# ilVecc/AquaticGymEnv

Hardware: AMD Instinct MI355X
Metric: env-steps/sec at batch=262144; achieved HBM GB/s vs roofline; 1/2/4/8-GPU scaling (higher is better)
Workload: dtype f32

## Files before the change

### aquaticgymenv_amd/csrc/aqua_hip.hip

```cpp
#include <hip/hip_runtime.h>
#include <hip/hip_ext.h>

#include <cmath>
#include <cstdarg>
#include <cstddef>
#include <type_traits>
#include <cstdio>
#include <cstring>
#include <vector>

#include "../../include/aqua_hip.h"
#include "aqua_device.hpp"

using namespace aqua;

namespace {

constexpr int TILE_WORLDS = 1024;
constexpr int BLOCK_SMALL = 256;
constexpr int RESET_GROUP = 8;
constexpr int MAX_GRID = 1 << 30;

constexpr size_t AQUA_BLOB_MIN_BYTES = 320;

struct StepArgs {
    float* state;
    int64_t ld;
    int32_t* time;
    const void* action;
    int64_t action_ld;
    const float* noise;
    int64_t noise_ld;
    float* reward;
    uint8_t* term;
    uint64_t* done_bits;
    float* obs_norm;
    const void* obst_blob;
    const uint64_t* tick_base;
    uint64_t seed, tick;
    int64_t N, env_offset;
    int64_t T, action_step_stride, out_step_stride;
    int64_t reseed_blocks;
    int K, waves, time_limit, auto_reset, random_boat, random_goal;
    float W, sigma;
    uint64_t* tick_copy_to;
    uint64_t* tick_bump_to;
    uint64_t tick_bump;
};

struct NsArgs {
    float* row[7];
    int32_t* time;
    const void* action;
    float* reward;
    uint8_t* term;
    uint64_t* done_bits;
    const void* obst_blob;
    const uint64_t* tick_base;
    uint64_t seed, tick;
    int64_t env_offset;
    uint32_t N, reseed_blocks;
    int32_t K, time_limit;
    float W, sigma;
    uint32_t flags;
    uint32_t reserved;
    const float* action_hi;
    const float* noise[2];
    float* norm[5];
    uint64_t* tick_copy_to;
    uint64_t* tick_bump_to;
    uint64_t tick_bump;
};
enum : uint32_t { NS_WAVES_MASK = 0xFFu, NS_RANDOM_BOAT = 1u << 8, NS_RANDOM_GOAL = 1u << 9, NS_HAS_NOISE = 1u << 10,
                  NS_HAS_NORM = 1u << 11, NS_DONE_WORD_WB = 1u << 12 };
constexpr int64_t NS_LAUNCH_MAX_WORLDS = int64_t(1) << 28;

__device__ __forceinline__ int args_waves(const StepArgs& a) { return a.waves; }
__device__ __forceinline__ int args_waves(const NsArgs& a) { return static_cast<int>(a.flags & NS_WAVES_MASK); }
__device__ __forceinline__ int args_random_boat(const StepArgs& a) { return a.random_boat; }
__device__ __forceinline__ int args_random_boat(const NsArgs& a) { return (a.flags & NS_RANDOM_BOAT) != 0; }
__device__ __forceinline__ int args_random_goal(const StepArgs& a) { return a.random_goal; }
__device__ __forceinline__ int args_random_goal(const NsArgs& a) { return (a.flags & NS_RANDOM_GOAL) != 0; }

template <typename T>
__device__ __forceinline__ T ld1(const T* p)
{
    return *p;
}
template <typename T>
__device__ __forceinline__ void st1(T* p, T v, bool wb = false)
{
#ifdef AQUA_ST1_PLAIN
    *p = v;
#else
    if (wb) *p = v;
    else __hip_atomic_store(p, v, __ATOMIC_RELAXED, __HIP_MEMORY_SCOPE_AGENT);
#endif
}

constexpr int64_t STORE_WB_SAME_STEP_MIN = int64_t(1) << 21;
constexpr int64_t STORE_WB_NEXT_STEP_MIN = int64_t(1) << 21, STORE_WB_NEXT_STEP_MAX = 3 * (int64_t(1) << 22);

constexpr int64_t DONE_WORD_WRITE_THROUGH_MAX_WORLDS = int64_t(1) << 20;
__device__ __forceinline__ void store_done_word(uint64_t* p, uint64_t v, int64_t n_worlds)
{
    if (n_worlds <= DONE_WORD_WRITE_THROUGH_MAX_WORLDS) st1(p, v);
    else *p = v;
}

template <typename T>
__device__ __forceinline__ T ld_at(const T* base, uint32_t byte_off)
{
    return ld1(reinterpret_cast<const T*>(reinterpret_cast<const char*>(base) + byte_off));
}
template <typename T>
__device__ __forceinline__ void st_at(T* base, uint32_t byte_off, T v, bool wb = false)
{
    st1(reinterpret_cast<T*>(reinterpret_cast<char*>(base) + byte_off), v, wb);
}

__device__ __forceinline__ ObstPtr obstacle_rows(const void* blob)
{
    return (ObstPtr)(uintptr_t)(static_cast<const char*>(blob) + sizeof(ObstHeader));
}

template <int QUICK = QUICK_NEVER, typename A>
__device__ __forceinline__ StepConst make_const(const A& a, ObstPtr obst)
{
    StepConst k;
    k.quick = nullptr;
    k.W = a.W; k.sigma = a.sigma; k.waves = args_waves(a); k.time_limit = a.time_limit; k.K = a.K;
    k.obst = obst;
    k.Kc = 0; k.band2 = 0.0f; k.band2_tight = 0.0f;
    k.touch[0] = k.touch[1] = k.touch[2] = k.touch[3] = 0;
    if (a.obst_blob != nullptr) {
        const ObstHeader __attribute__((address_space(4)))* h =
            (const ObstHeader __attribute__((address_space(4)))*)(uintptr_t)a.obst_blob;
        k.Kc = h->n_circles;
        k.band2 = h->band2;
        k.band2_tight = h->band2_tight;
        const uint32_t __attribute__((address_space(4)))* w = (const uint32_t __attribute__((address_space(4)))*)(uintptr_t)a.obst_blob;
        if (QUICK == QUICK_ALWAYS || (QUICK == QUICK_IF_PRESENT && a.K <= QUICK_MAX)) {
            k.quick = (QuickPtr)(uintptr_t)(reinterpret_cast<const char*>(a.obst_blob) + quick_offset(a.K));
            k.qc0 = quick_circles(k.quick, QUICK_C0);
            k.qr0 = quick_rects(k.quick, QUICK_R0);
        }
        k.touch[0] = w[16]; k.touch[1] = w[32]; k.touch[2] = w[48]; k.touch[3] = w[64];
    }
    k.obst64 = reinterpret_cast<const double*>(reinterpret_cast<const char*>(a.obst_blob) + sizeof(ObstHeader) +
                                               sizeof(ObstF) * a.K);
    return k;
}

__device__ __forceinline__ int fold_index(int64_t a)
{
    if (a < 0) a += 3;
    return a < 0 ? 0 : (a > 2 ? 2 : static_cast<int>(a));
}

struct Motion {
    float h, w, chord;
    float vl, vr;
    int idx;
};

// ... 448 lines not shown
    if (lane == 0) sh.count[parity][wave] = static_cast<uint32_t>(__builtin_popcountll(m));
    __syncthreads();
    uint32_t first = 0, total = 0;
#pragma unroll
    for (int w = 0; w < WAVES; ++w) {
        const uint32_t c = sh.count[parity][w];
        if (w < wave) first += c;
        total += c;
    }
    return ReseedTicket{uni(total), first + pos};
}

template <bool SMALL, typename A>
__device__ __forceinline__ void serve_reseed(const ReseedTicket& tk, const A& a, const StepConst& k, uint64_t tick,
                                             int64_t block_first_world, RolloutShared& sh, int parity)
{
    constexpr int WAVES = BLOCK_SMALL / 64;
    const int wave = threadIdx.x >> 6, lane = threadIdx.x & 63;
    if (tk.n == 0 || wave != static_cast<int>((static_cast<uint32_t>(tick) + blockIdx.x) & (WAVES - 1))) return;
#ifdef AQUA_FUSED_NOSERVE
    return;
#endif
    uint32_t first[WAVES + 1];
    first[0] = 0;
#pragma unroll
    for (int w = 0; w < WAVES; ++w) first[w + 1] = first[w] + sh.count[parity][w];
    constexpr uint32_t PER_PASS = 64 / RESET_GROUP;
    for (uint32_t qb = 0; qb < tk.n; qb += PER_PASS) {
        const uint32_t q = qb + (lane / RESET_GROUP);
        const bool active = q < tk.n;
        uint32_t seg = 0;
#pragma unroll
        for (int w = 1; w < WAVES; ++w) seg += (active && q >= first[w]) ? 1u : 0u;
        const uint32_t owner = sh.list[parity][seg][active ? q - first[seg] : 0];
        const uint64_t world = static_cast<uint64_t>(a.env_offset + block_first_world) + owner;
        EnvState f;
        if constexpr (SMALL)
            f = reset_env_group<RESET_GROUP, RESEED_QUICK>(active, a.seed, world, tick, k.waves, args_random_boat(a), args_random_goal(a),
                                                        k.K, k.obst, nullptr, k.quick, k.Kc);
        else
            f = reset_env_group<RESET_GROUP>(active, a.seed, world, tick, k.waves, args_random_boat(a), args_random_goal(a), k.K, k.obst);
        if (active && (lane & (RESET_GROUP - 1)) == 0) {
            float* r = sh.result[q];
            r[0] = f.x; r[1] = f.y; r[2] = f.th; r[3] = f.gx; r[4] = f.gy; r[5] = f.wx; r[6] = f.wy;
        }
    }
}

__device__ __forceinline__ void collect_reseed(EnvState& e, bool need, const ReseedTicket& tk, RolloutShared& sh)
{
    if (tk.n == 0) return;
    __syncthreads();
    if (need) {
        const float* r = sh.result[tk.slot];
        e.x = r[0]; e.y = r[1]; e.th = r[2]; e.gx = r[3]; e.gy = r[4]; e.wx = r[5]; e.wy = r[6]; e.t = 0;
    }
}

#ifndef AQUA_FUSED_MAIL
#define AQUA_FUSED_MAIL 1
#endif
#ifndef AQUA_MAIL_SPIN_LIMIT
#define AQUA_MAIL_SPIN_LIMIT (1u << 18)
#endif
constexpr uint32_t MAIL_SPIN_LIMIT = AQUA_MAIL_SPIN_LIMIT;
#ifndef AQUA_MAIL_PRIO
#define AQUA_MAIL_PRIO 2
#endif
struct RolloutMail {
    uint32_t posted[BLOCK_SMALL / 64];
    uint32_t served;
    uint32_t count[2][BLOCK_SMALL / 64];
    uint8_t list[2][BLOCK_SMALL / 64][64];
    float result[2][BLOCK_SMALL][8];
};

__device__ __forceinline__ uint32_t lds_offset(const void* p)
{
    return static_cast<uint32_t>(reinterpret_cast<uintptr_t>((const __attribute__((address_space(3))) void*)p));
}
__device__ __forceinline__ void mail_wait(const uint32_t* flag, uint32_t at_least)
{
    const uint32_t at = lds_offset(flag);
    for (uint32_t polls = 0; polls < MAIL_SPIN_LIMIT; ++polls) {
        uint32_t v;
        asm volatile("ds_read_b32 %0, %1\n\ts_waitcnt lgkmcnt(0)" : "=v"(v) : "v"(at) : "memory");
        if (uni(v) >= at_least) break;
        __builtin_amdgcn_s_sleep(1);
    }
}
__device__ __forceinline__ void mail_flag(uint32_t* flag, uint32_t value)
{
    asm volatile("s_waitcnt lgkmcnt(0)\n\tds_write_b32 %0, %1" ::"v"(lds_offset(flag)), "v"(value) : "memory");
}
__device__ __forceinline__ uint32_t mail_post(bool need, RolloutMail& sh, uint32_t q)
{
    const int wave = threadIdx.x >> 6, lane = threadIdx.x & 63, parity = static_cast<int>(q & 1u);
    if (q >= 2u) mail_wait(&sh.served, q - 1u);
    const uint64_t m = __ballot(need);
    const uint32_t pos = __builtin_amdgcn_mbcnt_hi(static_cast<uint32_t>(m >> 32), __builtin_amdgcn_mbcnt_lo(static_cast<uint32_t>(m), 0u));
    if (need) sh.list[parity][wave][pos] = static_cast<uint8_t>(lane);
    if (lane == 0) {
        sh.count[parity][wave] = static_cast<uint32_t>(__builtin_popcountll(m));
        mail_flag(&sh.posted[wave], q + 1u);
    }
    return pos;
}

template <bool SMALL, typename A>
__device__ __forceinline__ void mail_serve(const A& a, const StepConst& k, uint64_t tick, int64_t block_first_world, RolloutMail& sh, uint32_t q)
{
    constexpr int WAVES = BLOCK_SMALL / 64;
    const int lane = threadIdx.x & 63, parity = static_cast<int>(q & 1u);
    uint32_t first[WAVES + 1];
    first[0] = 0;
#pragma unroll
    for (int w = 0; w < WAVES; ++w) {
        mail_wait(&sh.posted[w], q + 1u);
        first[w + 1] = first[w] + sh.count[parity][w];
    }
#ifdef AQUA_FUSED_NOSERVE
    const uint32_t n = 0;
#else
    const uint32_t n = uni(first[WAVES]);
#endif
    constexpr uint32_t PER_PASS = 64 / RESET_GROUP;
    for (uint32_t qb = 0; qb < n; qb += PER_PASS) {
        const uint32_t i = qb + (lane / RESET_GROUP);
        const bool active = i < n;
        uint32_t seg = 0;
#pragma unroll
        for (int w = 1; w < WAVES; ++w) seg += (active && i >= first[w]) ? 1u : 0u;
        const uint32_t at = active ? i - first[seg] : 0u;
        const uint32_t owner = seg * 64u + sh.list[parity][seg][at];
        const uint64_t world = static_cast<uint64_t>(a.env_offset + block_first_world) + owner;
        EnvState f;
        if constexpr (SMALL)
            f = reset_env_group<RESET_GROUP, RESEED_QUICK>(active, a.seed, world, tick, k.waves, args_random_boat(a), args_random_goal(a),
                                                        k.K, k.obst, nullptr, k.quick, k.Kc);
        else
            f = reset_env_group<RESET_GROUP>(active, a.seed, world, tick, k.waves, args_random_boat(a), args_random_goal(a), k.K, k.obst);
        if (active && (lane & (RESET_GROUP - 1)) == 0) {
            float* r = sh.result[parity][seg * 64u + at];
            r[0] = f.x; r[1] = f.y; r[2] = f.th; r[3] = f.gx; r[4] = f.gy; r[5] = f.wx; r[6] = f.wy;
        }
    }
    if (lane == 0) mail_flag(&sh.served, q + 1u);
}

__device__ __forceinline__ void mail_collect(EnvState& e, bool need, uint32_t pos, RolloutMail& sh, uint32_t q)
{
    if (!any_lane(need)) return;
    mail_wait(&sh.served, q + 1u);
    if (need) {
        const float* r = sh.result[q & 1u][(threadIdx.x & ~63u) + pos];
        e.x = r[0]; e.y = r[1]; e.th = r[2]; e.gx = r[3]; e.gy = r[4]; e.wx = r[5]; e.wy = r[6];
    }
}

struct TileShared {
    uint32_t count[TILE_WORLDS / 64];
    uint16_t list[TILE_WORLDS / 64][64];
};

template <int AK, bool SMALL_TABLE, bool RESTART, bool WB = false>
__global__ __launch_bounds__(TILE_WORLDS) void step_kernel(const NsArgs a)
// ... 43 lines not shown
    }
    asm volatile("" : "+v"(tin[0]), "+v"(u0[0]), "+v"(u1[0]));
    hold_loads<1, AK>(x, y, th, gx, gy, wx, wy, araw, avl, avr);
    fold_actions<1, AK>(araw, aidx);
    if constexpr (AK == AQUA_ACT_BEARING) aidx[0] = bearing_action(x[0], y[0], th[0], gx[0], gy[0]);
    const float x0 = x[0], y0 = y[0], th0 = th[0], wx0 = wx[0], wy0 = wy[0];
    EnvState e{x[0], y[0], th[0], gx[0], gy[0], wx[0], wy[0], tin[0]};
    const Motion mo = decode_motion<AK>(k, aidx[0], avl[0], avr[0]);
    float rew;
    uint32_t code;
    asm volatile("" ::"s"(k.touch[0]), "s"(k.touch[1]), "s"(k.touch[2]), "s"(k.touch[3]));
    const bool knife = fast_step<false, QUICK>(e, mo.h, mo.w, mo.chord, u0[0], u1[0], k, rew, code) && valid;
    if (__builtin_expect(any_lane(knife), 0)) {
        if (knife) {
            const ExactOut o2 = exact_step(x0, y0, th0, gx[0], gy[0], wx0, wy0, e.t, exact_motion<AK>(mo), k.K, k.obst64,
                                           k.obst, k.band2, k.time_limit);
            e.x = o2.x; e.y = o2.y; e.th = o2.th; rew = o2.reward; code = o2.term;
        }
    }
    const bool done = valid && code != 0u;
    uint32_t s4 = o4, s1 = o;
    asm volatile("" : "+v"(s4), "+v"(s1));
    constexpr bool wb = WB;
    if (valid) {
        st_at(a.reward, s4, rew, wb);
        st_at(a.term, s1, static_cast<uint8_t>(code), wb);
    }
    const uint64_t done_ballot = __ballot(done);
    if (a.done_bits != nullptr) {
        const uint32_t word = (tile >> 6) + (uni(off) >> 6);
        if (word < ((a.N + 63u) >> 6) && lane == 0) {
            if (a.flags & NS_DONE_WORD_WB) a.done_bits[word] = done_ballot;
            else st1(a.done_bits + word, done_ballot);
        }
    }
    if (valid && !(RESTART && done)) {
        st_at(a.row[0], s4, e.x, wb); st_at(a.row[1], s4, e.y, wb); st_at(a.row[2], s4, e.th, wb);
        st_at(a.row[5], s4, e.wx, wb); st_at(a.row[6], s4, e.wy, wb);
        st_at(a.time, s4, e.t, wb);
        ns_write_norm(a, s4, e.x, e.y, e.th, gx[0], gy[0], wb);
    }
    if constexpr (RESTART) {
        __shared__ TileShared sh;
        constexpr int WAVES = TILE_WORLDS / 64;
        if (done) sh.list[wave][__builtin_amdgcn_mbcnt_hi(static_cast<uint32_t>(done_ballot >> 32),
                                __builtin_amdgcn_mbcnt_lo(static_cast<uint32_t>(done_ballot), 0u))] = static_cast<uint16_t>(off);
        if (lane == 0) sh.count[wave] = static_cast<uint32_t>(__builtin_popcountll(done_ballot));
        __syncthreads();
        uint32_t first[WAVES + 1];
        first[0] = 0;
#pragma unroll
        for (int w = 0; w < WAVES; ++w) first[w + 1] = first[w] + sh.count[w];
        const uint32_t n_done = uni(first[WAVES]);
        const int waves = args_waves(a), random_boat = args_random_boat(a), random_goal = args_random_goal(a);
        const uint64_t env_base = static_cast<uint64_t>(a.env_offset) + tile;
        constexpr uint32_t GROUPS = TILE_WORLDS / RESET_GROUP;
        for (uint32_t qb = static_cast<uint32_t>(wave) * (64 / RESET_GROUP); qb < n_done; qb += GROUPS) {
            const uint32_t q = qb + (lane / RESET_GROUP);
            const bool active = q < n_done;
            uint32_t seg = 0;
#pragma unroll
            for (int w = 1; w < WAVES; ++w) seg += (active && q >= first[w]) ? 1u : 0u;
            const uint32_t i = sh.list[seg][active ? q - first[seg] : 0];
            EnvState f;
            if constexpr (SMALL_TABLE)
                f = reset_env_group<RESET_GROUP, RESEED_QUICK>(active, a.seed, env_base + i, tick, waves, random_boat, random_goal,
                                                            k.K, k.obst, nullptr, k.quick, k.Kc);
            else
                f = reset_env_group<RESET_GROUP>(active, a.seed, env_base + i, tick, waves, random_boat, random_goal, k.K, k.obst);
            if (active && (lane & (RESET_GROUP - 1)) == 0) {
                const uint32_t i4 = (tile + i) * 4u;
                st_at(a.row[0], i4, f.x, wb); st_at(a.row[1], i4, f.y, wb); st_at(a.row[2], i4, f.th, wb);
                st_at(a.row[3], i4, f.gx, wb); st_at(a.row[4], i4, f.gy, wb);
                st_at(a.row[5], i4, f.wx, wb); st_at(a.row[6], i4, f.wy, wb);
                st_at(a.time, i4, f.t, wb);
                ns_write_norm(a, i4, f.x, f.y, f.th, f.gx, f.gy, wb);
            }
        }
    }
}

constexpr bool rollout_mail(int mode) { return AQUA_FUSED_MAIL && mode == AQUA_RESET_NEXT_STEP; }
constexpr int rollout_threads(int mode) { return rollout_mail(mode) ? BLOCK_SMALL + 64 : BLOCK_SMALL; }
template <int AK, bool SMALL, int MODE>
__global__ __launch_bounds__(rollout_threads(MODE), rollout_threads(MODE) / 64) void rollout_kernel(const StepArgs a)
{
    constexpr bool MAIL = rollout_mail(MODE);
    __shared__ typename std::conditional<MAIL, RolloutMail, RolloutShared>::type sh;
    if constexpr (MAIL) {
        if (threadIdx.x < BLOCK_SMALL / 64) sh.posted[threadIdx.x] = 0u;
        if (threadIdx.x == 0) sh.served = 0u;
        __syncthreads();
    }
    constexpr int QUICK = SMALL ? QUICK_ALWAYS : QUICK_NEVER;
    const uint64_t tick0 = launch_tick(a);
    const int64_t N = a.N, ld = a.ld;
    uint32_t q0 = 0;
    if constexpr (MAIL) {
        if (threadIdx.x >= BLOCK_SMALL) {
            StepConst k = make_const<QUICK_NEVER>(a, obstacle_rows(a.obst_blob));
            if constexpr (SMALL) k.quick = (QuickPtr)(uintptr_t)(reinterpret_cast<const char*>(a.obst_blob) + quick_offset(a.K));
            if (AQUA_MAIL_PRIO) __builtin_amdgcn_s_setprio(AQUA_MAIL_PRIO);
            for (int64_t bbase = static_cast<int64_t>(blockIdx.x) * BLOCK_SMALL; bbase < N;
                 bbase += static_cast<int64_t>(gridDim.x) * BLOCK_SMALL, q0 += static_cast<uint32_t>(a.T))
                for (int64_t p = 0; p < a.T; ++p)
                    mail_serve<SMALL>(a, k, tick0 + static_cast<uint64_t>(p), bbase, sh, q0 + static_cast<uint32_t>(p));
            return;
        }
    }
#ifdef AQUA_FUSED_QUICK_RESIDENT
    const StepConst k = make_const<SMALL ? QUICK_IF_PRESENT : QUICK_NEVER>(a, obstacle_rows(a.obst_blob));
#else
    StepConst k = make_const<QUICK_NEVER>(a, obstacle_rows(a.obst_blob));
    if constexpr (SMALL) k.quick = (QuickPtr)(uintptr_t)(reinterpret_cast<const char*>(a.obst_blob) + quick_offset(a.K));
#endif
    for (int64_t bbase = static_cast<int64_t>(blockIdx.x) * BLOCK_SMALL; bbase < N;
         bbase += static_cast<int64_t>(gridDim.x) * BLOCK_SMALL, q0 += static_cast<uint32_t>(a.T)) {
        const int64_t i = bbase + threadIdx.x;
        const bool valid = i < N;
        const int64_t ic = valid ? i : N - 1;
        EnvState e{a.state[0 * ld + ic], a.state[1 * ld + ic], a.state[2 * ld + ic], a.state[3 * ld + ic],
                   a.state[4 * ld + ic], a.state[5 * ld + ic], a.state[6 * ld + ic], a.time[ic]};
        const uint64_t env = static_cast<uint64_t>(a.env_offset + i);
        bool owed = false;
        uint32_t owed_pos = 0, posted_pos = 0;
        if constexpr (MAIL) posted_pos = mail_post(valid && e.t == done_code(tick0 - 1), sh, q0);
        for (int64_t s = 0; s < a.T; ++s) {
            const uint64_t tick = tick0 + static_cast<uint64_t>(s);
            const int parity = static_cast<int>(s & 1);
            bool pending = false, restart = false;
            ReseedTicket tk{0u, 0u};
            if constexpr (MODE == AQUA_RESET_NEXT_STEP) {
                if (e.t == restart_code(tick - 1)) e.t = 0;
                restart = valid && e.t == done_code(tick - 1);
                pending = valid && e.t < 0;
                if constexpr (!MAIL) {
                    tk = publish_reseed(restart, sh, parity);
                    serve_reseed<SMALL>(tk, a, k, tick, bbase, sh, parity);
                }
            }
            int idx = 2;
            float vl = 0.5f, vr = 0.5f;
            if constexpr (AK == AQUA_ACT_U8) idx = fold_index(static_cast<const uint8_t*>(a.action)[s * a.action_step_stride + ic]);
            if constexpr (AK == AQUA_ACT_I32) idx = fold_index(static_cast<const int32_t*>(a.action)[s * a.action_step_stride + ic]);
            if constexpr (AK == AQUA_ACT_I64) idx = fold_index(static_cast<const int64_t*>(a.action)[s * a.action_step_stride + ic]);
            if constexpr (AK == AQUA_ACT_F32X2) {
                const float* base = static_cast<const float*>(a.action) + s * a.action_step_stride;
                vl = base[ic]; vr = base[a.action_ld + ic];
            }
            uint64_t seed = a.seed;
#ifdef AQUA_FUSED_KEYS_LAUNDERED
            asm volatile("" : "+s"(seed));
#endif
            uint32_t w0[1], w1[1];
            pair_draws<1, false>(seed, env, tick, STREAM_STEP, w0, w1);
            const float u0 = u_pm1(w0[0]), u1 = u_pm1(w1[0]);
            if constexpr (AK >= AQUA_ACT_SAMPLE_D) {
                pair_draws<1, false>(seed, env, tick, STREAM_ACT, w0, w1);
                if constexpr (AK == AQUA_ACT_SAMPLE_D) idx = sample_discrete(w0[0]);
                else { vl = sample_thrust(w0[0]); vr = sample_thrust(w1[0]); }
            }
            if constexpr (MAIL) {
                if (s > 0) mail_collect(e, owed, owed_pos, sh, q0 + static_cast<uint32_t>(s) - 1u);
            }
            if constexpr (AK == AQUA_ACT_BEARING) idx = bearing_action(e.x, e.y, e.th, e.gx, e.gy);
            const Motion m = decode_motion<AK>(k, idx, vl, vr);
            const EnvState before = e;
            EnvState after = e;
            float rew;
            uint32_t code;
#ifndef AQUA_FUSED_QUICK_RESIDENT
            if constexpr (SMALL) {
                QuickPtr q = k.quick;
                asm volatile("" : "+s"(q));
                k.qc0 = quick_circles(q, QUICK_C0);
                k.qr0 = quick_rects(q, QUICK_R0);
            }
#endif
            const bool knife = fast_step<false, QUICK>(after, m.h, m.w, m.chord, u0, u1, k, rew, code) && valid && !pending;
            if (__builtin_expect(any_lane(knife), 0)) {
                if (knife) {
                    const ExactOut o = exact_step(before.x, before.y, before.th, before.gx, before.gy, before.wx,
                                                  before.wy, after.t, exact_motion<AK>(m), k.K, k.obst64, k.obst, k.band2,
                                                  k.time_limit);
                    after.x = o.x; after.y = o.y; after.th = o.th; rew = o.reward; code = o.term;
                }
            }
            if (pending) { rew = 0.0f; code = 0u; }
            else e = after;
            if (valid) {
                a.reward[s * a.out_step_stride + i] = rew;
                a.term[s * a.out_step_stride + i] = static_cast<uint8_t>(code);
            }
            const bool done = valid && code != 0u;
            if constexpr (MAIL) {
                if (restart) e.t = restart_code(tick);
                else if (done) e.t = done_code(tick);
                owed = restart; owed_pos = posted_pos;
                if (s + 1 < a.T) posted_pos = mail_post(valid && e.t == done_code(tick), sh, q0 + static_cast<uint32_t>(s) + 1u);
            } else if constexpr (MODE == AQUA_RESET_NEXT_STEP) {
                collect_reseed(e, restart, tk, sh);
                if (restart) e.t = restart_code(tick);
                else if (done) e.t = done_code(tick);
            } else if constexpr (MODE == AQUA_RESET_SAME_STEP) {
                const ReseedTicket t1 = publish_reseed(done, sh, parity);
                serve_reseed<SMALL>(t1, a, k, tick, bbase, sh, parity);
                collect_reseed(e, done, t1, sh);
            }
        }
        if constexpr (MAIL) mail_collect(e, owed, owed_pos, sh, q0 + static_cast<uint32_t>(a.T) - 1u);
        if (valid) {
            a.state[0 * ld + i] = e.x; a.state[1 * ld + i] = e.y; a.state[2 * ld + i] = e.th;
            a.state[3 * ld + i] = e.gx; a.state[4 * ld + i] = e.gy;
            a.state[5 * ld + i] = e.wx; a.state[6 * ld + i] = e.wy;
            a.time[i] = e.t;
        }
    }
}

constexpr int RESET_SCAN_ROWS = 4, RESET_SCAN = RESET_SCAN_ROWS * BLOCK_SMALL, RESET_DENSE = RESET_SCAN / 8;
struct ResetShared {
    uint32_t count[BLOCK_SMALL / 64];
    uint16_t list[BLOCK_SMALL / 64][RESET_SCAN_ROWS * 64];
};
struct TablesShared {
    uint32_t count[BLOCK_SMALL / 64];
    uint8_t list[BLOCK_SMALL / 64][64];
};
constexpr int HANDOFF_PER_WAVE = 8;
template <int KREG>
struct HandoffShared {
    uint32_t count[BLOCK_SMALL / 64];
    uint8_t world[BLOCK_SMALL / 64][HANDOFF_PER_WAVE];
    ObstF rows[BLOCK_SMALL / 64][HANDOFF_PER_WAVE][KREG];
};
#ifndef AQUA_SINK_SLOTS
#define AQUA_SINK_SLOTS 3
#endif
constexpr int SINK_SLOTS = AQUA_SINK_SLOTS;
constexpr int SINK_SPLIT_SHORT = 2, SINK_SPLIT_LONG = 4, SINK_SPLIT_LONG_MIN_ROWS = 24;
struct SinkShared {
    uint32_t count[BLOCK_SMALL / 64];
    uint8_t world[BLOCK_SMALL / 64][SINK_SLOTS];
    float rows[BLOCK_SMALL / 64][SINK_SLOTS][AQUA_MAX_OBSTACLES * 5];
};
struct NoShared {};
constexpr int TABLES_NEXT_STEP_TILE = 3;
constexpr int TABLES_KREG = 8, TABLES_KREG_WIDE = 16, TABLES_KREG_WIDE_MIN = 11;
template <int AK, int MODE, int KREG, int SINK_SPLIT = 2>
__device__ __forceinline__ void tables_step_block(const StepArgs& a, const float* __restrict__ t32, const double* __restrict__ t64,
                                                  int64_t tld, float band2, float band2_tight, int64_t tile)
{
    constexpr bool RESTART = MODE == AQUA_RESET_SAME_STEP;
    constexpr bool NS = MODE == AQUA_RESET_NEXT_STEP || MODE == TABLES_NEXT_STEP_TILE;
    constexpr bool SINK = MODE == TABLES_NEXT_STEP_TILE && KREG == 0;
#ifndef AQUA_TABLES_NO_REFETCH
    constexpr bool REFETCH = MODE == AQUA_RESET_SAME_STEP && KREG == 0 && SINK_SPLIT > 1;
#else
    constexpr bool REFETCH = false;
#endif
    __shared__ typename std::conditional<SINK || REFETCH, SinkShared, NoShared>::type ssh;
    const int64_t ld = a.ld, rem = a.N - tile;
    const int lane = threadIdx.x & 63;
    float* const row0 = a.state + tile;
    int32_t* const trow = a.time + tile;
    const uint32_t last = static_cast<uint32_t>(rem < BLOCK_SMALL ? rem - 1 : BLOCK_SMALL - 1);
    const uint32_t off = threadIdx.x;
    const bool valid = static_cast<int64_t>(off) < rem;
    const uint32_t o = off < last ? off : last;
    const uint32_t o4 = o * 4u;
    float x[1], y[1], th[1], gx[1], gy[1], wx[1], wy[1], u0[1] = {0.0f}, u1[1] = {0.0f}, avl[1] = {0.5f}, avr[1] = {0.5f};
    int64_t araw[1] = {2};
    int aidx[1] = {2};
    const int32_t tin = ld_at(trow, o4);
    x[0] = ld_at(row0 + 0 * ld, o4); y[0] = ld_at(row0 + 1 * ld, o4); th[0] = ld_at(row0 + 2 * ld, o4);
    gx[0] = ld_at(row0 + 3 * ld, o4); gy[0] = ld_at(row0 + 4 * ld, o4);
    wx[0] = ld_at(row0 + 5 * ld, o4); wy[0] = ld_at(row0 + 6 * ld, o4);
    if constexpr (AK == AQUA_ACT_U8) araw[0] = ld_at(static_cast<const uint8_t*>(a.action) + tile, o);
    else if constexpr (AK == AQUA_ACT_I32) araw[0] = ld_at(static_cast<const int32_t*>(a.action) + tile, o4);
    else if constexpr (AK == AQUA_ACT_I64) araw[0] = ld_at(static_cast<const int64_t*>(a.action) + tile, o * 8u);
    else if constexpr (AK == AQUA_ACT_F32X2) {
        avl[0] = ld_at(static_cast<const float*>(a.action) + tile, o4);
        avr[0] = ld_at(static_cast<const float*>(a.action) + a.action_ld + tile, o4);
    }
    ObstF rows[KREG > 0 ? KREG : 1];
    if constexpr (KREG > 0) {
#pragma unroll
        for (int j = 0; j < KREG; ++j) {
            const int jj = j < a.K ? j : a.K - 1;
            const float* const rb = t32 + (6 * jj) * tld + tile;
            rows[j].cx = ld_at(rb, o4); rows[j].cy = ld_at(rb + tld, o4); rows[j].hx = ld_at(rb + 2 * tld, o4);
            rows[j].hy = ld_at(rb + 3 * tld, o4); rows[j].r2 = ld_at(rb + 4 * tld, o4);
        }
    }
    StepConst k;
    k.W = a.W; k.sigma = a.sigma; k.waves = a.waves; k.time_limit = a.time_limit; k.K = a.K; k.Kc = 0;
    k.band2 = band2; k.band2_tight = band2_tight; k.obst = nullptr; k.obst64 = nullptr;
    k.touch[0] = k.touch[1] = k.touch[2] = k.touch[3] = 0;
// ... 972 lines not shown
    if (done_bits != nullptr && !aligned(done_bits, 8)) return fail(AQUA_E_ALIGN, "done_bits must be 8-byte aligned");
    if (auto_reset < 0 || auto_reset > 2) return fail(AQUA_E_INVALID, "auto_reset must be 0, 1 or 2");
    if (N == 0) return 0;
    a.action = action; a.action_ld = action_ld; a.noise = noise; a.noise_ld = noise_ld;
    a.reward = reward; a.term = term; a.done_bits = done_bits; a.obs_norm = obs_norm; a.auto_reset = auto_reset;
    if (obs_norm != nullptr && !aligned(obs_norm, 4)) return fail(AQUA_E_ALIGN, "obs_norm must be 4-byte aligned");
    const hipError_t e = launch_step_any(a, action_kind, static_cast<hipStream_t>(stream));
    return e == hipSuccess ? 0 : hip_fail(e, "aqua_step_f32 launch");
}

int aqua_reset_f32(const AquaParams* p, const void* obst_blob_dev, int K, int64_t N, int64_t env_offset,
                   float* state, int64_t ld, int32_t* time, const uint8_t* mask, uint64_t seed, uint64_t tick,
                   const uint64_t* tick_base_dev, void* stream)
{
    StepArgs a;
    const int rc = fill_args(a, p, obst_blob_dev, K, N, env_offset, state, ld, time, seed, tick, tick_base_dev);
    if (rc) return rc;
    if (N == 0) return 0;
    hipLaunchKernelGGL(reset_kernel, dim3(grid_for(N, BLOCK_SMALL, 2048)), dim3(BLOCK_SMALL), 0, static_cast<hipStream_t>(stream), a, mask);
    const hipError_t e = hipGetLastError();
    return e == hipSuccess ? 0 : hip_fail(e, "aqua_reset_f32 launch");
}

int aqua_rollout_f32(const AquaParams* p, const void* obst_blob_dev, int K, int64_t N, int64_t env_offset,
                     float* state, int64_t ld, int32_t* time, int64_t T, const void* actions, int action_kind,
                     int64_t action_ld, int64_t action_step_stride, uint64_t seed, uint64_t tick,
                     const uint64_t* tick_base_dev, float* reward, uint8_t* term, int64_t out_step_stride,
                     uint64_t* done_bits, int64_t done_step_stride, float* obs_norm, int auto_reset, int advance_tick,
                     void* stream)
{
    return aqua_rollout_events_f32(p, obst_blob_dev, K, N, env_offset, state, ld, time, T, actions, action_kind, action_ld,
                                   action_step_stride, seed, tick, tick_base_dev, reward, term, out_step_stride, done_bits,
                                   done_step_stride, obs_norm, auto_reset, advance_tick, nullptr, nullptr, stream);
}

int aqua_rollout_events_f32(const AquaParams* p, const void* obst_blob_dev, int K, int64_t N, int64_t env_offset,
                            float* state, int64_t ld, int32_t* time, int64_t T, const void* actions, int action_kind,
                            int64_t action_ld, int64_t action_step_stride, uint64_t seed, uint64_t tick,
                            const uint64_t* tick_base_dev, float* reward, uint8_t* term, int64_t out_step_stride,
                            uint64_t* done_bits, int64_t done_step_stride, float* obs_norm, int auto_reset, int advance_tick,
                            AquaEvent* first_start, AquaEvent* last_stop, void* stream)
{
    StepArgs a;
    int rc = fill_args(a, p, obst_blob_dev, K, N, env_offset, state, ld, time, seed, tick, tick_base_dev);
    if (rc) return rc;
    rc = check_step_buffers(N, actions, action_kind, action_ld, nullptr, 0, reward, term);
    if (rc) return rc;
    if (T < 0 || action_step_stride < 0 || out_step_stride < 0 || done_step_stride < 0)
        return fail(AQUA_E_INVALID, "negative T or stride");
    if (auto_reset < 0 || auto_reset > 2) return fail(AQUA_E_INVALID, "auto_reset must be 0, 1 or 2");
    if (advance_tick && tick_base_dev == nullptr) return fail(AQUA_E_INVALID, "advance_tick needs tick_base_dev");
    if (N == 0 || T == 0) return 0;
    a.action_ld = action_ld; a.auto_reset = auto_reset; a.obs_norm = obs_norm;
    const size_t esz = action_elem_bytes(action_kind);
    uint64_t* const tick_words = const_cast<uint64_t*>(tick_base_dev);
    for (int64_t t = 0; t < T; ++t) {
        a.tick = tick + static_cast<uint64_t>(t);
        if (advance_tick && T >= 2) {
            a.tick_base = (t == T - 1) ? tick_words + 1 : tick_words;
            a.tick_copy_to = (t == 0) ? tick_words + 1 : nullptr;
            a.tick_bump_to = (t == T - 1) ? tick_words : nullptr;
            a.tick_bump = static_cast<uint64_t>(T);
        }
        a.action = actions ? static_cast<const char*>(actions) + static_cast<size_t>(t * action_step_stride) * esz : nullptr;
        a.reward = reward + t * out_step_stride;
        a.term = term + t * out_step_stride;
        a.done_bits = done_bits ? done_bits + t * done_step_stride : nullptr;
        LaunchEvents ev;
        if (t == 0 && first_start != nullptr) ev.start = first_start->event;
        if (t == T - 1 && last_stop != nullptr) ev.stop = last_stop->event;
        const hipError_t e = launch_step_any(a, action_kind, static_cast<hipStream_t>(stream), ev);
        if (e != hipSuccess) return hip_fail(e, "aqua_rollout_f32 launch");
    }
    if (advance_tick && T == 1) return aqua_tick_advance(tick_words, 1, stream);
    return 0;
}

int aqua_rollout_fused_f32(const AquaParams* p, const void* obst_blob_dev, int K, int64_t N, int64_t env_offset,
                           float* state, int64_t ld, int32_t* time, int64_t T, const void* actions,
                           int action_kind, int64_t action_ld, int64_t action_step_stride, uint64_t seed,
                           uint64_t tick, const uint64_t* tick_base_dev, float* reward, uint8_t* term,
                           int64_t out_step_stride, int auto_reset, void* stream)
{
    StepArgs a;
    int rc = fill_args(a, p, obst_blob_dev, K, N, env_offset, state, ld, time, seed, tick, tick_base_dev);
    if (rc) return rc;
    rc = check_step_buffers(N, actions, action_kind, action_ld, nullptr, 0, reward, term);
    if (rc) return rc;
    if (T < 0 || action_step_stride < 0 || out_step_stride < 0) return fail(AQUA_E_INVALID, "negative T or stride");
    if (auto_reset < 0 || auto_reset > 2) return fail(AQUA_E_INVALID, "auto_reset must be 0, 1 or 2");
    if (N == 0 || T == 0) return 0;
    a.action = actions; a.action_ld = action_ld; a.action_step_stride = action_step_stride;
    a.reward = reward; a.term = term; a.out_step_stride = out_step_stride; a.T = T; a.auto_reset = auto_reset;
    const dim3 grid(grid_for(N, BLOCK_SMALL, 2048)), block(rollout_threads(auto_reset));
    hipStream_t s = static_cast<hipStream_t>(stream);
    const bool small = K > 0 && K <= QUICK_MAX;
#define AQUA_ROLLOUT_MODE(AK, SM)                                                                                         \
    do {                                                                                                                  \
        if (auto_reset == AQUA_RESET_NEXT_STEP) hipLaunchKernelGGL((rollout_kernel<AK, SM, AQUA_RESET_NEXT_STEP>), grid, block, 0, s, a); \
        else if (auto_reset == AQUA_RESET_SAME_STEP) hipLaunchKernelGGL((rollout_kernel<AK, SM, AQUA_RESET_SAME_STEP>), grid, block, 0, s, a); \
        else hipLaunchKernelGGL((rollout_kernel<AK, SM, 0>), grid, block, 0, s, a);                                       \
    } while (0)
#define AQUA_ROLLOUT_LAUNCH(AK)                                                                      \
    case AK:                                                                                         \
        if (small) AQUA_ROLLOUT_MODE(AK, true);                                                      \
        else AQUA_ROLLOUT_MODE(AK, false);                                                           \
        break;
    switch (action_kind) {
        AQUA_ROLLOUT_LAUNCH(AQUA_ACT_U8)
        AQUA_DEV_OTHER_KINDS(AQUA_ROLLOUT_LAUNCH)
#undef AQUA_ROLLOUT_LAUNCH
#undef AQUA_ROLLOUT_MODE
        default: return fail(AQUA_E_INVALID, "unknown action_kind %d", action_kind);
    }
    const hipError_t e = hipGetLastError();
    return e == hipSuccess ? 0 : hip_fail(e, "aqua_rollout_fused_f32 launch");
}

size_t aqua_tables32_floats(int K, int64_t tld)
{
    return (K < 1 || tld < 0) ? 0 : static_cast<size_t>(12) * static_cast<size_t>(K) * static_cast<size_t>(tld);
}

int aqua_pack_tables(const double* rows, int K, int64_t N, int64_t tld, float* tab32_host, double* tab64_host, float* r_max_out)
{
    if (K < 1 || K > AQUA_MAX_OBSTACLES) return fail(AQUA_E_INVALID, "K=%d outside [1, %d]", K, AQUA_MAX_OBSTACLES);
    if (N < 0 || tld < N) return fail(AQUA_E_INVALID, "bad sizes: N=%lld tld=%lld", (long long)N, (long long)tld);
    if (rows == nullptr || tab32_host == nullptr || tab64_host == nullptr || r_max_out == nullptr)
        return fail(AQUA_E_INVALID, "rows/tab32/tab64/r_max is NULL");
    const auto tight = [](double R) {
        return 2.5 * (R + static_cast<double>(BAND)) * static_cast<double>(BAND_TIGHT) + 4.0 * 1.1920929e-7 * R * R;
    };
    double r_max = 2.5;
    for (int64_t i = 0; i < N; ++i)
        for (int k = 0; k < K; ++k) {
            const double* o = rows + (i * K + k) * 5;
            if (o[2] < 0.0) continue;
            if (!(o[2] == 0.0 || o[2] == 1.0)) return fail(AQUA_E_INVALID, "world %lld obstacle %d: kind must be 0, 1 or < 0", (long long)i, k);
            if (o[3] < 0.0 || (o[2] == 1.0 && o[4] < 0.0)) return fail(AQUA_E_INVALID, "world %lld obstacle %d: negative size", (long long)i, k);
            if (o[2] == 0.0 && 2.5 + o[3] > r_max) r_max = 2.5 + o[3];
        }
    const float b_max = static_cast<float>(tight(r_max));
    for (int64_t i = 0; i < N; ++i)
        for (int k = 0; k < K; ++k) {
            const double* o = rows + (i * K + k) * 5;
            float* f = tab32_host + (6 * k) * tld + i;
            double* d = tab64_host + (5 * k) * tld + i;
            for (int c = 0; c < 5; ++c) d[c * tld] = o[c];
            if (o[2] < 0.0) {
                f[0] = f[tld] = f[2 * tld] = f[3 * tld] = 0.0f; f[4 * tld] = -3.0e38f; f[5 * tld] = 1.0f;
                continue;
            }
            double hx = 0, hy = 0, R = 2.5;
            if (o[2] == 0.0) R += o[3]; else { hx = o[3] / 2; hy = o[4] / 2; }
            f[0] = static_cast<float>(o[0]); f[tld] = static_cast<float>(o[1]);
            f[2 * tld] = static_cast<float>(hx); f[3 * tld] = static_cast<float>(hy);
            const float r2 = static_cast<float>(R * R);
            f[4 * tld] = r2;
            f[5 * tld] = static_cast<float>(static_cast<double>(b_max) /
                                            tight_rounded(std::sqrt(static_cast<double>(r2)), geometry_rounding(o)));
        }
    float* const aos = tab32_host + static_cast<size_t>(6) * K * tld;
    for (int64_t i = 0; i < N; ++i)
        for (int k = 0; k < K; ++k)
            for (int c = 0; c < 6; ++c) aos[(i * K + k) * 6 + c] = tab32_host[(6 * k + c) * tld + i];
    *r_max_out = static_cast<float>(r_max);
    return 0;
}

namespace {
int fill_table_args(StepArgs& a, const AquaParams* p, const float* tab32, int K, int64_t tld, int64_t N, int64_t env_offset,
                    float* state, int64_t ld, int32_t* time, uint64_t seed, uint64_t tick, const uint64_t* tick_base)
{
    if (K < 1) return fail(AQUA_E_INVALID, "K=%d: per-world tables need at least one row", K);
    if (tab32 == nullptr) return fail(AQUA_E_INVALID, "tab32 is NULL");
    if (tld < N) return fail(AQUA_E_INVALID, "tld=%lld < N=%lld", (long long)tld, (long long)N);
// ... 451 lines not shown
```

Before: 54.23 billion.

## Slim fused rollout kernel args and lazily reload pointers from kernarg segment

Replaces StepArgs in the fused rollout kernel with a compact RolloutArgs whose row pointers, step byte strides, obst64 and action_hi pointers are re-read from the kernarg segment on demand. It also switches indexing to 32-bit offsets, bumps per-step pointers instead of recomputing 64-bit products, and raises launch bounds to 5 waves. The aim is to cut SGPR/VGPR pressure and 64-bit address arithmetic so occupancy rises. It adds limits on N and T per call and more scalar kernarg loads inside the step loop.

```diff
diff --git a/aquaticgymenv_amd/csrc/aqua_hip.hip b/aquaticgymenv_amd/csrc/aqua_hip.hip
--- a/aquaticgymenv_amd/csrc/aqua_hip.hip
+++ b/aquaticgymenv_amd/csrc/aqua_hip.hip
@@ -75,12 +75,43 @@
                   NS_HAS_NORM = 1u << 11, NS_DONE_WORD_WB = 1u << 12 };
 constexpr int64_t NS_LAUNCH_MAX_WORLDS = int64_t(1) << 28;
 
+struct RolloutRows {
+    float* row[7];
+    int32_t* time;
+};
+struct RolloutArgs {
+    const void* action;
+    float* reward;
+    uint8_t* term;
+    const void* obst_blob;
+    uint64_t seed, tick;
+    int64_t env_offset;
+    uint32_t N, T;
+    int32_t K, time_limit;
+    float W, sigma;
+    uint32_t flags;
+    uint32_t reserved;
+    RolloutRows rows;
+    const float* action_hi;
+    const uint64_t* tick_base;
+    int64_t action_step_bytes, reward_step_bytes, term_step_bytes;
+    uint64_t* tick_copy_to;
+    uint64_t* tick_bump_to;
+    uint64_t tick_bump;
+};
+enum : uint32_t { RO_HAS_TICK_BASE = 1u << 16 };
+static_assert(std::is_standard_layout<RolloutArgs>::value, "offsetof() into the kernel-argument segment needs a standard-layout struct");
+constexpr int64_t ROLLOUT_MAX_STEPS = (int64_t(1) << 31) - 1;
+
 __device__ __forceinline__ int args_waves(const StepArgs& a) { return a.waves; }
 __device__ __forceinline__ int args_waves(const NsArgs& a) { return static_cast<int>(a.flags & NS_WAVES_MASK); }
+__device__ __forceinline__ int args_waves(const RolloutArgs& a) { return static_cast<int>(a.flags & NS_WAVES_MASK); }
 __device__ __forceinline__ int args_random_boat(const StepArgs& a) { return a.random_boat; }
 __device__ __forceinline__ int args_random_boat(const NsArgs& a) { return (a.flags & NS_RANDOM_BOAT) != 0; }
+__device__ __forceinline__ int args_random_boat(const RolloutArgs& a) { return (a.flags & NS_RANDOM_BOAT) != 0; }
 __device__ __forceinline__ int args_random_goal(const StepArgs& a) { return a.random_goal; }
 __device__ __forceinline__ int args_random_goal(const NsArgs& a) { return (a.flags & NS_RANDOM_GOAL) != 0; }
+__device__ __forceinline__ int args_random_goal(const RolloutArgs& a) { return (a.flags & NS_RANDOM_GOAL) != 0; }
 
 template <typename T>
 __device__ __forceinline__ T ld1(const T* p)
@@ -695,6 +726,7 @@
 __device__ __forceinline__ void mail_wait(const uint32_t* flag, uint32_t at_least)
 {
     const uint32_t at = lds_offset(flag);
+#pragma unroll 1
     for (uint32_t polls = 0; polls < MAIL_SPIN_LIMIT; ++polls) {
         uint32_t v;
         asm volatile("ds_read_b32 %0, %1\n\ts_waitcnt lgkmcnt(0)" : "=v"(v) : "v"(at) : "memory");
@@ -904,8 +936,56 @@
 
 constexpr bool rollout_mail(int mode) { return AQUA_FUSED_MAIL && mode == AQUA_RESET_NEXT_STEP; }
 constexpr int rollout_threads(int mode) { return rollout_mail(mode) ? BLOCK_SMALL + 64 : BLOCK_SMALL; }
+template <bool SMALL>
+__device__ __forceinline__ StepConst rollout_const(const RolloutArgs& a)
+{
+    StepConst k;
+    k.W = a.W; k.sigma = a.sigma; k.waves = args_waves(a); k.time_limit = a.time_limit; k.K = a.K;
+    k.obst = obstacle_rows(a.obst_blob);
+    k.quick = nullptr;
+    k.Kc = 0; k.band2 = 0.0f; k.band2_tight = 0.0f;
+    k.touch[0] = k.touch[1] = k.touch[2] = k.touch[3] = 0;
+    if (SMALL || a.K > 0) {
+        const ObstHeader __attribute__((address_space(4)))* h =
+            (const ObstHeader __attribute__((address_space(4)))*)(uintptr_t)a.obst_blob;
+        k.Kc = h->n_circles;
+        k.band2 = h->band2;
+        k.band2_tight = h->band2_tight;
+    }
+    if constexpr (SMALL) k.quick = (QuickPtr)(uintptr_t)(reinterpret_cast<const char*>(a.obst_blob) + quick_offset(a.K));
+    k.obst64 = nullptr;
+    return k;
+}
+__device__ __forceinline__ const double* rollout_obst64()
+{
+    const char* const blob = kernarg_at<const char*>(offsetof(RolloutArgs, obst_blob));
+    const int K = kernarg_at<int32_t>(offsetof(RolloutArgs, K));
+    return reinterpret_cast<const double*>(blob + sizeof(ObstHeader) + sizeof(ObstF) * K);
+}
+__device__ __forceinline__ RolloutRows rollout_rows()
+{
+    using KernArg = const char __attribute__((address_space(4)))*;
+    KernArg kp = (KernArg)__builtin_amdgcn_kernarg_segment_ptr();
+    asm volatile("" : "+s"(kp));
+    kp += offsetof(RolloutArgs, rows);
+    RolloutRows r;
+#pragma unroll
+    for (int j = 0; j < 7; ++j) r.row[j] = *(float* const __attribute__((address_space(4)))*)(kp + offsetof(RolloutRows, row) + sizeof(float*) * j);
+    r.time = *(int32_t* const __attribute__((address_space(4)))*)(kp + offsetof(RolloutRows, time));
+    return r;
+}
+__device__ __forceinline__ uint64_t rollout_tick(const RolloutArgs& a)
+{
+    if (!(a.flags & RO_HAS_TICK_BASE)) return a.tick;
+    return a.tick + *(const uint64_t __attribute__((address_space(4)))*)(uintptr_t)kernarg_at<const uint64_t*>(offsetof(RolloutArgs, tick_base));
+}
+
+#ifndef AQUA_FUSED_SAME_STEP_WAVES
+#define AQUA_FUSED_SAME_STEP_WAVES 5
+#endif
+constexpr int rollout_waves(int mode) { return mode == AQUA_RESET_SAME_STEP ? AQUA_FUSED_SAME_STEP_WAVES : 5; }
 template <int AK, bool SMALL, int MODE>
-__global__ __launch_bounds__(rollout_threads(MODE), rollout_threads(MODE) / 64) void rollout_kernel(const StepArgs a)
+__global__ __launch_bounds__(rollout_threads(MODE), rollout_waves(MODE)) void rollout_kernel(const RolloutArgs a)
 {
     constexpr bool MAIL = rollout_mail(MODE);
     __shared__ typename std::conditional<MAIL, RolloutMail, RolloutShared>::type sh;
@@ -915,41 +995,55 @@
         __syncthreads();
     }
     constexpr int QUICK = SMALL ? QUICK_ALWAYS : QUICK_NEVER;
-    const uint64_t tick0 = launch_tick(a);
-    const int64_t N = a.N, ld = a.ld;
+    const uint32_t N = a.N, T = a.T;
+    const uint32_t tile_stride = gridDim.x * BLOCK_SMALL;
     uint32_t q0 = 0;
     if constexpr (MAIL) {
         if (threadIdx.x >= BLOCK_SMALL) {
-            StepConst k = make_const<QUICK_NEVER>(a, obstacle_rows(a.obst_blob));
-            if constexpr (SMALL) k.quick = (QuickPtr)(uintptr_t)(reinterpret_cast<const char*>(a.obst_blob) + quick_offset(a.K));
+            const StepConst k = rollout_const<SMALL>(a);
+            const uint64_t tick0 = rollout_tick(a);
             if (AQUA_MAIL_PRIO) __builtin_amdgcn_s_setprio(AQUA_MAIL_PRIO);
-            for (int64_t bbase = static_cast<int64_t>(blockIdx.x) * BLOCK_SMALL; bbase < N;
-                 bbase += static_cast<int64_t>(gridDim.x) * BLOCK_SMALL, q0 += static_cast<uint32_t>(a.T))
-                for (int64_t p = 0; p < a.T; ++p)
-                    mail_serve<SMALL>(a, k, tick0 + static_cast<uint64_t>(p), bbase, sh, q0 + static_cast<uint32_t>(p));
+            for (uint32_t bbase = blockIdx.x * BLOCK_SMALL; bbase < N; bbase += tile_stride, q0 += T)
+                for (uint32_t p = 0; p < T; ++p)
+                    mail_serve<SMALL>(a, k, tick0 + p, static_cast<int64_t>(bbase), sh, q0 + p);
             return;
         }
     }
 #ifdef AQUA_FUSED_QUICK_RESIDENT
-    const StepConst k = make_const<SMALL ? QUICK_IF_PRESENT : QUICK_NEVER>(a, obstacle_rows(a.obst_blob));
+    StepConst k = make_const<SMALL ? QUICK_IF_PRESENT : QUICK_NEVER>(a, obstacle_rows(a.obst_blob));
 #else
-    StepConst k = make_const<QUICK_NEVER>(a, obstacle_rows(a.obst_blob));
-    if constexpr (SMALL) k.quick = (QuickPtr)(uintptr_t)(reinterpret_cast<const char*>(a.obst_blob) + quick_offset(a.K));
+    StepConst k = rollout_const<SMALL>(a);
 #endif
-    for (int64_t bbase = static_cast<int64_t>(blockIdx.x) * BLOCK_SMALL; bbase < N;
-         bbase += static_cast<int64_t>(gridDim.x) * BLOCK_SMALL, q0 += static_cast<uint32_t>(a.T)) {
-        const int64_t i = bbase + threadIdx.x;
+    const uint64_t tick0 = rollout_tick(a);
+    for (uint32_t bbase = blockIdx.x * BLOCK_SMALL; bbase < N; bbase += tile_stride, q0 += T) {
+        const uint32_t i = bbase + threadIdx.x;
         const bool valid = i < N;
-        const int64_t ic = valid ? i : N - 1;
-        EnvState e{a.state[0 * ld + ic], a.state[1 * ld + ic], a.state[2 * ld + ic], a.state[3 * ld + ic],
-                   a.state[4 * ld + ic], a.state[5 * ld + ic], a.state[6 * ld + ic], a.time[ic]};
-        const uint64_t env = static_cast<uint64_t>(a.env_offset + i);
+        uint32_t o = valid ? i : N - 1u;
+        EnvState e;
+        {
+            const RolloutRows r = rollout_rows();
+            e.x = ld_at(r.row[0], o * 4u); e.y = ld_at(r.row[1], o * 4u); e.th = ld_at(r.row[2], o * 4u); e.gx = ld_at(r.row[3], o * 4u);
+            e.gy = ld_at(r.row[4], o * 4u); e.wx = ld_at(r.row[5], o * 4u); e.wy = ld_at(r.row[6], o * 4u); e.t = ld_at(r.time, o * 4u);
+        }
+        uint64_t env = static_cast<uint64_t>(a.env_offset) + i;
+        const char* act = static_cast<const char*>(a.action);
+        const char* act_hi = nullptr;
+        if constexpr (AK == AQUA_ACT_F32X2) act_hi = kernarg_at<const char*>(offsetof(RolloutArgs, action_hi));
+        char* rew_row = reinterpret_cast<char*>(a.reward);
+        uint8_t* term_row = a.term;
         bool owed = false;
         uint32_t owed_pos = 0, posted_pos = 0;
         if constexpr (MAIL) posted_pos = mail_post(valid && e.t == done_code(tick0 - 1), sh, q0);
-        for (int64_t s = 0; s < a.T; ++s) {
-            const uint64_t tick = tick0 + static_cast<uint64_t>(s);
-            const int parity = static_cast<int>(s & 1);
+        for (uint32_t s = 0; s < T; ++s) {
+            const uint64_t tick = tick0 + s;
+            if constexpr (MODE == AQUA_RESET_SAME_STEP) {
+                uint32_t lane_world = threadIdx.x;
+                asm volatile("" : "+v"(lane_world));
+                lane_world += bbase;
+                env = static_cast<uint64_t>(a.env_offset) + lane_world;
+                o = lane_world < N ? lane_world : N - 1u;
+            }
+            const int parity = static_cast<int>(s & 1u);
             bool pending = false, restart = false;
             ReseedTicket tk{0u, 0u};
             if constexpr (MODE == AQUA_RESET_NEXT_STEP) {
@@ -958,17 +1052,17 @@
                 pending = valid && e.t < 0;
                 if constexpr (!MAIL) {
                     tk = publish_reseed(restart, sh, parity);
-                    serve_reseed<SMALL>(tk, a, k, tick, bbase, sh, parity);
+                    serve_reseed<SMALL>(tk, a, k, tick, static_cast<int64_t>(bbase), sh, parity);
                 }
             }
             int idx = 2;
             float vl = 0.5f, vr = 0.5f;
-            if constexpr (AK == AQUA_ACT_U8) idx = fold_index(static_cast<const uint8_t*>(a.action)[s * a.action_step_stride + ic]);
-            if constexpr (AK == AQUA_ACT_I32) idx = fold_index(static_cast<const int32_t*>(a.action)[s * a.action_step_stride + ic]);
-            if constexpr (AK == AQUA_ACT_I64) idx = fold_index(static_cast<const int64_t*>(a.action)[s * a.action_step_stride + ic]);
+            if constexpr (AK == AQUA_ACT_U8) idx = fold_index(ld_at(reinterpret_cast<const uint8_t*>(act), o));
+            if constexpr (AK == AQUA_ACT_I32) idx = fold_index(ld_at(reinterpret_cast<const int32_t*>(act), o * 4u));
+            if constexpr (AK == AQUA_ACT_I64) idx = fold_index(ld_at(reinterpret_cast<const int64_t*>(act), o * 8u));
             if constexpr (AK == AQUA_ACT_F32X2) {
-                const float* base = static_cast<const float*>(a.action) + s * a.action_step_stride;
-                vl = base[ic]; vr = base[a.action_ld + ic];
+                vl = ld_at(reinterpret_cast<const float*>(act), o * 4u);
+                vr = ld_at(reinterpret_cast<const float*>(act_hi), o * 4u);
             }
             uint64_t seed = a.seed;
 #ifdef AQUA_FUSED_KEYS_LAUNDERED
@@ -983,7 +1077,7 @@
                 else { vl = sample_thrust(w0[0]); vr = sample_thrust(w1[0]); }
             }
             if constexpr (MAIL) {
-                if (s > 0) mail_collect(e, owed, owed_pos, sh, q0 + static_cast<uint32_t>(s) - 1u);
+                if (s > 0) mail_collect(e, owed, owed_pos, sh, q0 + s - 1u);
             }
             if constexpr (AK == AQUA_ACT_BEARING) idx = bearing_action(e.x, e.y, e.th, e.gx, e.gy);
             const Motion m = decode_motion<AK>(k, idx, vl, vr);
@@ -1002,40 +1096,45 @@
             const bool knife = fast_step<false, QUICK>(after, m.h, m.w, m.chord, u0, u1, k, rew, code) && valid && !pending;
             if (__builtin_expect(any_lane(knife), 0)) {
                 if (knife) {
-                    const ExactOut o = exact_step(before.x, before.y, before.th, before.gx, before.gy, before.wx,
-                                                  before.wy, after.t, exact_motion<AK>(m), k.K, k.obst64, k.obst, k.band2,
+                    const ExactOut x = exact_step(before.x, before.y, before.th, before.gx, before.gy, before.wx,
+                                                  before.wy, after.t, exact_motion<AK>(m), k.K, rollout_obst64(), k.obst, k.band2,
                                                   k.time_limit);
-                    after.x = o.x; after.y = o.y; after.th = o.th; rew = o.reward; code = o.term;
+                    after.x = x.x; after.y = x.y; after.th = x.th; rew = x.reward; code = x.term;
                 }
             }
             if (pending) { rew = 0.0f; code = 0u; }
             else e = after;
             if (valid) {
-                a.reward[s * a.out_step_stride + i] = rew;
-                a.term[s * a.out_step_stride + i] = static_cast<uint8_t>(code);
+                st_at(reinterpret_cast<float*>(rew_row), o * 4u, rew, true);
+                st_at(term_row, o, static_cast<uint8_t>(code), true);
             }
+            act += kernarg_at<int64_t>(offsetof(RolloutArgs, action_step_bytes));
+            if constexpr (AK == AQUA_ACT_F32X2) act_hi += kernarg_at<int64_t>(offsetof(RolloutArgs, action_step_bytes));
+            rew_row += kernarg_at<int64_t>(offsetof(RolloutArgs, reward_step_bytes));
+            term_row += kernarg_at<int64_t>(offsetof(RolloutArgs, term_step_bytes));
             const bool done = valid && code != 0u;
             if constexpr (MAIL) {
                 if (restart) e.t = restart_code(tick);
                 else if (done) e.t = done_code(tick);
                 owed = restart; owed_pos = posted_pos;
-                if (s + 1 < a.T) posted_pos = mail_post(valid && e.t == done_code(tick), sh, q0 + static_cast<uint32_t>(s) + 1u);
+                if (s + 1u < T) posted_pos = mail_post(valid && e.t == done_code(tick), sh, q0 + s + 1u);
             } else if constexpr (MODE == AQUA_RESET_NEXT_STEP) {
                 collect_reseed(e, restart, tk, sh);
                 if (restart) e.t = restart_code(tick);
                 else if (done) e.t = done_code(tick);
             } else if constexpr (MODE == AQUA_RESET_SAME_STEP) {
                 const ReseedTicket t1 = publish_reseed(done, sh, parity);
-                serve_reseed<SMALL>(t1, a, k, tick, bbase, sh, parity);
+                serve_reseed<SMALL>(t1, a, k, tick, static_cast<int64_t>(bbase), sh, parity);
                 collect_reseed(e, done, t1, sh);
             }
         }
-        if constexpr (MAIL) mail_collect(e, owed, owed_pos, sh, q0 + static_cast<uint32_t>(a.T) - 1u);
+        if constexpr (MAIL) mail_collect(e, owed, owed_pos, sh, q0 + T - 1u);
         if (valid) {
-            a.state[0 * ld + i] = e.x; a.state[1 * ld + i] = e.y; a.state[2 * ld + i] = e.th;
-            a.state[3 * ld + i] = e.gx; a.state[4 * ld + i] = e.gy;
-            a.state[5 * ld + i] = e.wx; a.state[6 * ld + i] = e.wy;
-            a.time[i] = e.t;
+            const RolloutRows r = rollout_rows();
+            st_at(r.row[0], o * 4u, e.x, true); st_at(r.row[1], o * 4u, e.y, true); st_at(r.row[2], o * 4u, e.th, true);
+            st_at(r.row[3], o * 4u, e.gx, true); st_at(r.row[4], o * 4u, e.gy, true);
+            st_at(r.row[5], o * 4u, e.wx, true); st_at(r.row[6], o * 4u, e.wy, true);
+            st_at(r.time, o * 4u, e.t, true);
         }
     }
 }
@@ -2174,16 +2273,34 @@
                            uint64_t tick, const uint64_t* tick_base_dev, float* reward, uint8_t* term,
                            int64_t out_step_stride, int auto_reset, void* stream)
 {
-    StepArgs a;
-    int rc = fill_args(a, p, obst_blob_dev, K, N, env_offset, state, ld, time, seed, tick, tick_base_dev);
+    StepArgs a0;
+    int rc = fill_args(a0, p, obst_blob_dev, K, N, env_offset, state, ld, time, seed, tick, tick_base_dev);
     if (rc) return rc;
     rc = check_step_buffers(N, actions, action_kind, action_ld, nullptr, 0, reward, term);
     if (rc) return rc;
     if (T < 0 || action_step_stride < 0 || out_step_stride < 0) return fail(AQUA_E_INVALID, "negative T or stride");
     if (auto_reset < 0 || auto_reset > 2) return fail(AQUA_E_INVALID, "auto_reset must be 0, 1 or 2");
     if (N == 0 || T == 0) return 0;
-    a.action = actions; a.action_ld = action_ld; a.action_step_stride = action_step_stride;
-    a.reward = reward; a.term = term; a.out_step_stride = out_step_stride; a.T = T; a.auto_reset = auto_reset;
+    if (N > NS_LAUNCH_MAX_WORLDS)
+        return fail(AQUA_E_INVALID, "N=%lld: a fused rollout takes at most %lld worlds per call", (long long)N, (long long)NS_LAUNCH_MAX_WORLDS);
+    if (T > ROLLOUT_MAX_STEPS)
+        return fail(AQUA_E_INVALID, "T=%lld: a fused rollout takes at most %lld steps per call", (long long)T, (long long)ROLLOUT_MAX_STEPS);
+    RolloutArgs a;
+    std::memset(&a, 0, sizeof(a));
+    const int64_t esz = static_cast<int64_t>(action_elem_bytes(action_kind));
+    a.action = actions; a.reward = reward; a.term = term;
+    a.obst_blob = a0.obst_blob; a.seed = a0.seed; a.tick = a0.tick; a.env_offset = a0.env_offset;
+    a.N = static_cast<uint32_t>(N); a.T = static_cast<uint32_t>(T);
+    a.K = a0.K; a.time_limit = a0.time_limit; a.W = a0.W; a.sigma = a0.sigma;
+    a.flags = (static_cast<uint32_t>(a0.waves) & NS_WAVES_MASK) | (a0.random_boat ? NS_RANDOM_BOAT : 0u) | (a0.random_goal ? NS_RANDOM_GOAL : 0u) |
+              (tick_base_dev != nullptr ? RO_HAS_TICK_BASE : 0u);
+    for (int r = 0; r < 7; ++r) a.rows.row[r] = state + r * ld;
+    a.rows.time = time;
+    a.action_hi = (action_kind == AQUA_ACT_F32X2) ? static_cast<const float*>(actions) + action_ld : nullptr;
+    a.tick_base = tick_base_dev;
+    a.action_step_bytes = action_step_stride * esz;
+    a.reward_step_bytes = out_step_stride * static_cast<int64_t>(sizeof(float));
+    a.term_step_bytes = out_step_stride;
     const dim3 grid(grid_for(N, BLOCK_SMALL, 2048)), block(rollout_threads(auto_reset));
     hipStream_t s = static_cast<hipStream_t>(stream);
     const bool small = K > 0 && K <= QUICK_MAX;
```

Result: no change. 54.41 billion (median of 3 runs) (+0.3%).
